# FofanovLab/mtsv_tools

Measured on AMD Instinct MI355X. Metric: reads/sec (whole node), 150bp reads vs MG-index, higher is better.
Workload: dtype u32/i16

## Files before the change

mtsv_tools_amd/csrc/batch.hip:

```cpp
#include <atomic>
#include <chrono>
#include <cmath>
#include <condition_variable>
#include <exception>
#include <mutex>
#include <thread>
#include <cstdio>
#include <cstdlib>
#include <cstring>
#include <stdexcept>
#include <vector>

#include "../../include/mtsv_amd.h"
#include "batch.hpp"
#include "kernels.hpp"

namespace mtsv {

namespace {
template <class F>
void parallel_ranges(uint64_t n, F f) {
    static const int max_nt = [] {
        const char* e = getenv("MTSV_COPY_THREADS");
        return e ? std::max(1, std::min(16, atoi(e))) : 4;
// ... 102 lines not shown
    dev_alloc(&d_out_off, ns + 1, &bytes);
    dev_alloc(&d_tile_sums, (uint64_t)scan_tiles((uint32_t)ns) + 1, &bytes);
    dev_alloc(&d_counters, kCounters, &bytes);
    alloc_hit_workspace();
    dev_alloc(&d_hits, hits_cap, &bytes);
    HIP_CHECK(hipHostMalloc((void**)&h_counters, kCounters * sizeof(uint64_t), hipHostMallocMapped));
    if (const char* e = getenv("MTSV_SW")) sw_pairs = strcmp(e, "packed") != 0;
    if (const char* e = getenv("MTSV_SW_DIAG")) sw_diag = atoi(e) != 0;
    if (const char* e = getenv("MTSV_SW_PREPASS")) sw_prepass = atoi(e) != 0;
    if (const char* e = getenv("MTSV_SW_TOP")) sw_top = atoi(e) != 0;
    if (const char* e = getenv("MTSV_SW_BOUND")) sw_bound = atoi(e) != 0;
    if (const char* e = getenv("MTSV_SW_FUSED")) sw_fused = atoi(e) != 0;
    verify_mode = g_default_verify_mode;
    if (const char* e = getenv("MTSV_VERIFY")) verify_mode = !strcmp(e, "edit_first") ? 1 : 0;
    for (auto& e : ev) HIP_CHECK(hipEventCreate(&e));
    for (int k = 1; k < n_lanes; k++) {
        extra.emplace_back(new Batch(ix, di, ws_reads, 0, hit_cap_user, this));
        bytes += extra.back()->bytes;
    }
}

Batch::~Batch() {
    extra.clear();
    (void)hipSetDevice(di->device);
    (void)hipStreamSynchronize(stream);
    for (void* p : {(void*)d_bases, (void*)d_read_off, (void*)d_seed_lo, (void*)d_seed_cnt, (void*)d_seed_pre, (void*)d_strand_hits,
                    (void*)d_strand_nseeds, (void*)d_strand_off, (void*)d_strand_ncand, (void*)d_worklist,
                    (void*)d_strand_nout, (void*)d_out_off, (void*)d_tile_sums, (void*)d_counters, (void*)d_hit_row,
                    (void*)d_hit_ref, (void*)d_hit_q, (void*)d_hit_key, (void*)d_cand_tmp, (void*)d_cand, (void*)d_out,
                    (void*)d_hits, (void*)d_cand_next, (void*)d_cand_status, (void*)d_heavy_list})
        (void)hipFree(p);
    (void)hipFree(d_codes);
    (void)hipFree(d_strip);
    if (h_hits_stage) pinned_hits_release(h_hits_stage);
    if (copy_stream2) (void)hipStreamDestroy(copy_stream2);
    if (copy_stream) {
        (void)hipStreamSynchronize(copy_stream);
        (void)hipStreamDestroy(copy_stream);
    }
    for (auto& ar : arena) {
        (void)hipFree(ar.d_bases);
        (void)hipFree(ar.d_packed);
        (void)hipFree(ar.d_off);
    }
    if (h_off_all) (void)hipHostFree(h_off_all);
    for (auto& hs : h_stage)
        if (hs) (void)hipHostFree(hs);
    for (auto& e : chunk_ev) (void)hipEventDestroy(e);
    (void)hipHostFree(h_counters);
    for (auto& e : ev) (void)hipEventDestroy(e);
    (void)hipStreamDestroy(stream);
}

void Batch::alloc_hit_workspace() {
    dev_alloc(&d_hit_row, hit_cap, &bytes);
    dev_alloc(&d_hit_ref, hit_cap, &bytes);
    dev_alloc(&d_hit_q, hit_cap, &bytes);
    dev_alloc(&d_hit_key, hit_cap, &bytes);
    dev_alloc(&d_cand_tmp, 2 * hit_cap, &bytes);
    dev_alloc(&d_cand, hit_cap, &bytes);
    dev_alloc(&d_out, hit_cap, &bytes);
    dev_alloc(&d_cand_next, hit_cap, &bytes);
    dev_alloc(&d_cand_status, hit_cap, &bytes);
    dev_alloc(&d_worklist, hit_cap, &bytes);
}

// ... 219 lines not shown
    while (r0 < n_slice) {
        uint32_t nr = (uint32_t)std::min<uint64_t>(pass_reads, n_slice - r0);
        uint32_t pass_max_len = slice_max_len;
        bool tiled = false;
        if (mixed) {
            auto len_of = [&](uint64_t i) { return h_off[i + 1] - h_off[i]; };
            tiled = len_of(r0) > kMaxRegisterReadLen;
            uint32_t cnt = 0, ml = 0;
            while (cnt < nr && (len_of(r0 + cnt) > kMaxRegisterReadLen) == tiled) {
                const uint32_t ml2 = std::max(ml, len_of(r0 + cnt));
                if (tiled && cnt && 2ull * (cnt + 1) * (ml2 >= K ? (ml2 - K) / G + 1 : 0) > kLongPassSlots) break;
                ml = ml2;
                cnt++;
            }
            nr = cnt;
            pass_max_len = ml;
        }
        const uint32_t max_ns = pass_max_len >= K ? (pass_max_len - K) / G + 1 : 0;
        const uint32_t nstr = nr * 2;
        const uint64_t slots = (uint64_t)nstr * max_ns;
        if (slots > seed_cap) {
            (void)hipFree(d_seed_lo);
            (void)hipFree(d_seed_cnt);
            (void)hipFree(d_seed_pre);
            d_seed_lo = d_seed_cnt = d_seed_pre = nullptr;
            const uint64_t want = tiled ? slots : std::max<uint64_t>(slots, 2 * ws_reads * (uint64_t)max_ns);
            uint64_t dummy = 0;
            if (getenv("MTSV_TRACE")) fprintf(stderr, "[workspace] seed slot arrays grow %llu -> %llu entries\n", (unsigned long long)seed_cap, (unsigned long long)want);
            dev_alloc(&d_seed_lo, want, &dummy);
            dev_alloc(&d_seed_cnt, want, &dummy);
            dev_alloc(&d_seed_pre, want, &dummy);
            seed_cap = want;
        }
        HIP_CHECK(hipEventRecord(ev[0], stream));
        const uint32_t listed_cap = (uint32_t)std::min<uint64_t>(slots, std::max<uint64_t>(4096, (uint64_t)((double)slots * listed_share)));
        launch_search(stream, v, sb, so, (uint32_t)r0, nr, max_ns, K, G, d_seed_lo, d_seed_cnt, d_seed_pre, (uint32_t*)(d_counters + 22), listed_cap);
        HIP_CHECK(hipEventRecord(ev[1], stream));
        if (max_ns)
            launch_thin(stream, sb, so, (uint32_t)r0, nr, p.edit_rate, p.min_seed, max_ns, K, G, p.max_hits, p.tune_max_hits, d_seed_cnt,
                        d_seed_pre, d_strand_hits, d_strand_nseeds);
        else {
            HIP_CHECK(hipMemsetAsync(d_strand_hits, 0, (uint64_t)nstr * 4, stream));
            HIP_CHECK(hipMemsetAsync(d_strand_nseeds, 0, (uint64_t)nstr * 4, stream));
        }
        launch_scan(stream, d_strand_hits, nstr, d_tile_sums, d_counters + 0, d_strand_off);
        launch_publish(stream, d_counters, h_counters, 1);
        launch_publish(stream, d_counters + 22, h_counters + 22, 1);
        HIP_CHECK(hipEventRecord(ev[2], stream));
        HIP_CHECK(hipStreamSynchronize(stream));
        {
            const uint64_t n_listed = h_counters[22] & 0xffffffffull;
            const double share = slots ? (double)n_listed / (double)slots : 0.0;
            if (n_listed > listed_cap) {
                listed_share = std::min(1.0, share * 1.25 + 0.01);
                if (getenv("MTSV_TRACE")) fprintf(stderr, "[lane] %llu listed seed slots, grid for %u: pass again\n", (unsigned long long)n_listed, listed_cap);
                continue;
            }
            listed_share = std::min(1.0, std::max(0.02, share * 1.5 + 0.005));
        }
        const uint64_t total_hits = h_counters[0];
        if (total_hits > hit_cap) {
            if (nr > 1) {
                pass_reads = std::max<uint64_t>(1, nr / 2);
                continue;
            }
            if (total_hits > 0xfffffff0ull)
                throw std::runtime_error("device: one read has " + std::to_string(total_hits) + " seed hits, more than 2^32");
            grow_hit_workspace(total_hits);
        }
        stats.n_passes++;
        stats.n_seed_slots += slots;
        stats.n_seed_hits += total_hits;
        launch_expand(stream, v, nstr, max_ns, G, d_seed_lo, d_seed_cnt, d_seed_pre, d_strand_off, d_hit_row, d_hit_ref,
                      d_hit_q);
        HIP_CHECK(hipEventRecord(ev[3], stream));
        if (!v.sa_full)
            launch_locate(stream, v, (uint32_t)total_hits, d_strand_off + nstr, d_hit_row, d_hit_ref,
                          (unsigned long long*)(d_counters + 2));
        HIP_CHECK(hipEventRecord(ev[4], stream));
        HIP_CHECK(hipMemsetAsync(d_counters + 1, 0, 8, stream));
        HIP_CHECK(hipMemsetAsync(d_counters + 7, 0, 8, stream));
        HIP_CHECK(hipMemsetAsync(d_counters + 15, 0, 8, stream));
        launch_coalesce(stream, v, so, (uint32_t)r0, nstr, p.max_candidates, d_strand_off,
                        d_strand_nseeds, d_hit_ref, d_hit_q, d_hit_key, d_cand_tmp, d_cand, d_cand_next,
                        d_cand_status, d_strand_ncand, d_worklist, d_heavy_list, d_counters);
        HIP_CHECK(hipEventRecord(ev[5], stream));
        {
            EvalArgs a;
            a.bases = sb;
            a.read_off = so;
            a.r0 = (uint32_t)r0;
            a.edit_rate = p.edit_rate;
            a.max_candidates = p.max_candidates;
            a.strand_off = d_strand_off;
            a.cand = d_cand;
            a.cand_next = d_cand_next;
            a.cand_status = d_cand_status;
            a.out = d_out;
            a.n_verified = (unsigned long long*)(d_counters + 4);
            a.window_bytes = (unsigned long long*)(d_counters + 5);
            a.sw_columns = (unsigned long long*)(d_counters + 14);
            a.worklist = d_worklist;
            a.wl_count = (const uint32_t*)(d_counters + 1);
            a.wl_cursor = (uint32_t*)(d_counters + 7);
            stats.n_rounds = 1;
            if (tiled) {
                HIP_CHECK(hipMemsetAsync(d_counters + 13, 0, sizeof(uint64_t), stream));
                launch_max_window(stream, nstr, d_strand_off, d_strand_ncand, d_cand, (unsigned long long*)(d_counters + 13));
                launch_publish(stream, d_counters + 13, h_counters + 13, 1);
                HIP_CHECK(hipStreamSynchronize(stream));
                const uint32_t strip_len = (uint32_t)std::max<uint64_t>(h_counters[13], 1);
                const uint64_t need = (uint64_t)tiled_groups(total_hits, strip_len) * strip_len;
                if (need > strip_cap) {
                    (void)hipFree(d_strip);
                    d_strip = nullptr;
                    uint64_t dummy = 0;
                    dev_alloc(&d_strip, need, &dummy);
                    strip_cap = need;
                }
                a.strip = d_strip;
                a.strip_len = strip_len;
                launch_evaluate_tiled(stream, v, a, total_hits);
            } else if (verify_mode == 1 && pass_max_len <= 253) {
                launch_edit_myers(stream, v, a, total_hits, pass_max_len);
            } else if (sw_pairs && pass_max_len <= 253 && hit_cap < 0x80000000ull) {
                const bool fused = sw_bound && sw_fused;
                uint32_t* pass_list = (uint32_t*)d_hit_key;
                uint32_t* sweep_list = (uint32_t*)d_hit_key + hit_cap;
                uint32_t* next_lists[2] = {(uint32_t*)d_cand_tmp, (uint32_t*)d_cand_tmp + hit_cap};
                const uint32_t* wl = d_worklist;
// ... 711 lines not shown
```

mtsv_tools_amd/csrc/batch.hpp:

```cpp
#pragma once
#include <memory>
#include <mutex>
#include <vector>

#include "../../include/mtsv_amd.h"
#include "host_pack.hpp"
#include "dev_index.hpp"
#include "kernels.hpp"

namespace mtsv {

struct Batch {
    mtsv_index* ix;
    DeviceIndex* di;
    hipStream_t stream = nullptr, copy_stream2 = nullptr;
    mtsv_hit* h_hits_stage = nullptr;
    uint64_t h_hits_cap = 0, staged_hits = 0, last_total_hits = 0;
    bool staged_valid = false;
    struct Arena {
        uint8_t* d_bases = nullptr;
        uint8_t* d_packed = nullptr;
        uint32_t* d_off = nullptr;
        uint64_t cap_bases = 0, cap_reads = 0;
    };
// ... 8 lines not shown
    std::vector<hipEvent_t> chunk_ev;
    std::mutex* commit_mu = nullptr;
    uint64_t max_reads, max_bases, hit_cap, hits_cap = 0;
    uint64_t bytes = 0;
    Batch* parent = nullptr;
    std::vector<std::unique_ptr<Batch>> extra;
    int n_lanes = 1;
    uint64_t ws_reads = 0;
    struct Segment {
        Batch* lane;
        uint64_t offset, count;
    };
    std::vector<Segment> segments;
    uint64_t total_hits = 0;
    double run_t0 = 0;
    uint64_t lanes_used = 1;

    uint8_t* d_codes = nullptr;
    uint8_t* d_bases = nullptr;
    uint32_t* d_read_off = nullptr;
    uint32_t *d_seed_lo = nullptr, *d_seed_cnt = nullptr, *d_seed_pre = nullptr;
    uint64_t seed_cap = 0;
    uint32_t *d_strand_hits = nullptr, *d_strand_nseeds = nullptr, *d_strand_off = nullptr, *d_strand_ncand = nullptr,
             *d_worklist = nullptr, *d_strand_nout = nullptr, *d_out_off = nullptr;
    uint64_t* d_tile_sums = nullptr;
    uint64_t* d_counters = nullptr;
    uint32_t *d_hit_row = nullptr, *d_hit_ref = nullptr, *d_hit_q = nullptr;
    uint64_t *d_hit_key = nullptr, *d_cand_tmp = nullptr;
    uint4 *d_cand = nullptr, *d_out = nullptr;
    uint32_t *d_cand_next = nullptr, *d_cand_status = nullptr, *d_heavy_list = nullptr;
    DevHit* d_hits = nullptr;
    uint2* d_strip = nullptr;
    uint64_t strip_cap = 0;
    uint64_t* h_counters = nullptr;
    hipEvent_t ev[15];
    float sw_ms_acc = 0, sweep_ms_acc = 0, diag_ms_acc = 0, bound_ms_acc = 0, edit_ms_acc = 0;
    uint64_t sw_passed_acc = 0;

    std::vector<uint32_t> h_read_off;
    uint32_t max_len = 0;
    static constexpr int kCounters = 24;
    double listed_share = 0.125;
    bool sw_diag = true;
    bool sw_top = true;
    bool sw_bound = true;
    bool sw_fused = true;
    bool sw_prepass = true;
    bool sw_pairs = true;
    int verify_mode = 0;
    uint64_t n_reads = 0;
    uint64_t n_hits_total = 0;
    mtsv_batch_stats stats{};
    float stage_acc[MTSV_N_STAGES] = {0};

    Batch(mtsv_index* ix, DeviceIndex* di, uint64_t max_reads, uint64_t max_bases, uint64_t hit_cap, Batch* parent = nullptr, int lanes = 0);
    ~Batch();
    Batch(const Batch&) = delete;
    Batch& operator=(const Batch&) = delete;

    void upload(const uint8_t* bases, const uint64_t* read_off, uint64_t n);
    void run(const mtsv_params& p);
    void run_host(const uint8_t* bases, const uint64_t* read_off, uint64_t n, const mtsv_params& p, uint64_t read_base = 0);
    struct HostPart {
        const uint8_t* bases;
        const uint64_t* read_off;
        uint64_t n;
// ... 40 lines not shown
```

mtsv_tools_amd/csrc/k_seed.hip:

```cpp
#include "kernels_common.hpp"

namespace mtsv {

namespace {

__device__ inline uint32_t fast_code(uint32_t ch);
__global__ __launch_bounds__(256) void k_normalise(const uint8_t* src, uint8_t* dst, uint64_t lo, uint64_t hi) {
    const uint64_t i = (lo & ~15ull) + ((uint64_t)blockIdx.x * blockDim.x + threadIdx.x) * 16;
    if (i >= hi) return;
    if (i < lo || i + 16 > hi) {
        const uint64_t a = i < lo ? lo : i, b = i + 16 > hi ? hi : i + 16;
        for (uint64_t q = a; q < b; q++) dst[q] = (uint8_t)fast_code(src[q]);
        return;
    }
    uint4 v = *reinterpret_cast<const uint4*>(src + i);
    uint32_t w[4] = {v.x, v.y, v.z, v.w};
#pragma unroll
    for (int k = 0; k < 4; k++) {
        uint32_t o = 0;
#pragma unroll
        for (int q = 0; q < 4; q++) o |= fast_code((w[k] >> (8 * q)) & 0xffu) << (8 * q);
        w[k] = o;
    }
    *reinterpret_cast<uint4*>(dst + i) = make_uint4(w[0], w[1], w[2], w[3]);
// ... 329 lines not shown
        }
    }
    __syncthreads();
    uint32_t at = 0;
    if (lane == 0 && n_slow) at = atomicAdd(&tail_n, n_slow);
    at = __builtin_amdgcn_readfirstlane(at);
    if (lane < n_slow) tail_q[at + lane] = slow_q[lane];
    __syncthreads();
    const uint32_t nt = tail_n;
    if (nt) {
        __shared__ uint32_t tail_base;
        if (threadIdx.x == 0) tail_base = atomicAdd(slow_count, nt);
        __syncthreads();
        if (threadIdx.x < nt) slow_list[tail_base + threadIdx.x] = tail_q[threadIdx.x];
    }
}

__global__ __launch_bounds__(256) void k_search_listed(DevIndexView ix, const uint8_t* __restrict__ bases,
                                                       const uint32_t* __restrict__ read_off, uint32_t r0, uint32_t max_ns, uint32_t K,
                                                       uint32_t G, const uint32_t* __restrict__ slow_list,
                                                       const uint32_t* __restrict__ slow_count, uint32_t* __restrict__ seed_lo,
                                                       uint32_t* __restrict__ seed_cnt) {
    const uint32_t i = blockIdx.x * blockDim.x + threadIdx.x;
    if (i >= *slow_count) return;
    search_slot(ix, bases, read_off, r0, max_ns, K, G, slow_list[i], seed_lo, seed_cnt);
}


__global__ __launch_bounds__(256) void k_thin(const uint8_t* __restrict__ bases, const uint32_t* __restrict__ read_off,
                                              uint32_t r0, uint32_t n_reads, double edit_rate, double min_seed,
                                              uint32_t max_ns, uint32_t K, uint32_t G, uint64_t max_hits,
                                              uint64_t tune_max_hits, uint32_t* __restrict__ seed_cnt,
                                              uint32_t* __restrict__ seed_pre, uint32_t* __restrict__ strand_hits,
                                              uint32_t* __restrict__ strand_nseeds) {
    uint32_t rs = blockIdx.x * blockDim.x + threadIdx.x;
    if (rs >= n_reads * 2) return;
    uint32_t r = r0 + (rs >> 1);
    const uint32_t b0 = read_off[r];
    uint32_t L = read_off[r + 1] - b0;
    uint32_t ns = n_seeds_of(L, K, G);
    uint64_t next_offset = 0, seed_interval = G;
    uint32_t total = 0, nseeds = 0;
    uint32_t* cnt = seed_cnt + (uint64_t)rs * max_ns;
    uint32_t* pre = seed_pre + (uint64_t)rs * max_ns;
    for (uint32_t j = 0; j < ns; j++) {
        uint64_t offset = (uint64_t)j * G;
        const uint32_t raw = cnt[j];
        const uint32_t c = raw == kSeedAtPos ? 1u : raw;
        if (offset < next_offset) {
            if (c) cnt[j] = 0;
            continue;
        }
        if (c == 0) continue;
        if ((uint64_t)c > max_hits) {
            cnt[j] = 0;
            continue;
        }
        if ((uint64_t)c > tune_max_hits) {
            seed_interval *= 2;
            next_offset = offset + seed_interval;
        }
        pre[j] = total;
        total += c;
        nseeds++;
    }
    {
        const bool need = total != 0;
        const int other_need = __shfl_xor((int)need, 1);
        const bool pair_need = need || other_need != 0;
        const uint32_t ED = (uint32_t)ceil((double)L * edit_rate);
        bool hopeless = 2ull * ED > (uint64_t)L;
        uint32_t nn = 0;
        if (pair_need && !hopeless) {
            const uint4* b128 = reinterpret_cast<const uint4*>(bases);
            const uint32_t q0 = b0 >> 4, q1 = (b0 + L + 15) >> 4;
            auto masked = [&](uint32_t qi) {
                const uint4 v = b128[qi];
                const uint32_t w[4] = {v.x, v.y, v.z, v.w};
                uint32_t cnt = 0;
#pragma unroll
                for (int k = 0; k < 4; k++) {
                    const uint32_t byte0 = qi * 16 + 4 * k;
                    uint32_t m = (w[k] >> 2) & 0x01010101u;
                    const int lo = (int)b0 - (int)byte0, hi = (int)(b0 + L) - (int)byte0;
                    if (lo > 0) m = lo >= 4 ? 0u : (m & (0xffffffffu << (8 * lo)));
                    if (hi < 4) m = hi <= 0 ? 0u : (m & ((1u << (8 * hi)) - 1u));
                    cnt += __popc(m);
                }
                return cnt;
            };
            const uint32_t half = rs & 1, ng = q1 - q0;
            if (ng >= 1 && half == 0) nn += masked(q0);
            if (ng >= 2 && half == ((ng - 1) & 1)) nn += masked(q1 - 1);
            for (uint32_t g = half ? 1 : 2; g + 1 < ng; g += 2) {
                const uint4 v = b128[q0 + g];
                nn += __popc((v.x >> 2) & 0x01010101u) + __popc((v.y >> 2) & 0x01010101u) + __popc((v.z >> 2) & 0x01010101u) +
                      __popc((v.w >> 2) & 0x01010101u);
            }
        }
        nn += (uint32_t)__shfl_xor((int)nn, 1);
        hopeless = hopeless || nn > ED;
        const double ms = floor((double)nseeds * min_seed);
        const uint32_t min_seeds = ms < 1.0 ? 1u : (ms > 65535.0 ? 65535u : (uint32_t)ms);
        nseeds = min_seeds | (ED << 16) | ((need && hopeless) ? kHopeless : 0u);
    }
    strand_hits[rs] = total;
    strand_nseeds[rs] = nseeds;
}

constexpr int kScanThreads = 256;
constexpr int kScanItems = 8;
constexpr int kScanTile = kScanThreads * kScanItems;

__device__ inline uint32_t wave_incl_scan(uint32_t v) {
    for (int d = 1; d < kWave; d <<= 1) {
        uint32_t o = __shfl_up(v, d);
        if ((int)lane_id() >= d) v += o;
    }
    return v;
}

__global__ __launch_bounds__(kScanThreads) void k_scan_tile_sums(const uint32_t* __restrict__ in, uint32_t n,
                                                                 uint64_t* __restrict__ tile_sums) {
    __shared__ uint32_t ws[kScanThreads / kWave];
    uint32_t base = blockIdx.x * kScanTile + threadIdx.x * kScanItems;
    uint32_t s = 0;
    for (int i = 0; i < kScanItems; i++)
        if (base + i < n) s += in[base + i];
    for (int d = 32; d > 0; d >>= 1) s += __shfl_down(s, d);
    if (lane_id() == 0) ws[threadIdx.x / kWave] = s;
// ... 186 lines not shown
    (void)hipMemsetAsync(slow_count, 0, sizeof(uint32_t), s);
    uint64_t total = (uint64_t)n_reads * 2 * max_ns;
    if (!total) return;
    const bool fast = ix.kmer_tab && total < 0xffffffffull && K >= 16 && K <= 24 && ix.kmer_k >= 12 && ix.kmer_k <= 17 &&
                      K >= ix.kmer_k && K - std::min<uint32_t>(ix.kmer_k, 16) <= 8 && !getenv("MTSV_SEARCH_GENERIC");
    if (!fast) {
        hipLaunchKernelGGL(k_search, dim3(cdiv(total, 256)), dim3(256), 0, s, ix, bases, read_off, r0, n_reads, max_ns, K, G,
                           seed_lo, seed_cnt);
        return;
    }
    const dim3 grid(std::min<uint32_t>(cdiv(total, 256), 256 * 16));
#define FAST_CASE(KKV)                                                                                                  \
    if (K - KKV > 2)                                                                                                    \
        hipLaunchKernelGGL((k_search_fast<KKV, true>), grid, dim3(256), 0, s, ix, bases, read_off, r0, (uint32_t)total, max_ns, K, G, \
                           seed_lo, seed_cnt, slow_list, slow_count);                                                   \
    else                                                                                                                \
        hipLaunchKernelGGL((k_search_fast<KKV, false>), grid, dim3(256), 0, s, ix, bases, read_off, r0, (uint32_t)total, max_ns, K, G, \
                           seed_lo, seed_cnt, slow_list, slow_count)
    switch (ix.kmer_k) {
    case 12: FAST_CASE(12); break;
    case 13: FAST_CASE(13); break;
    case 14: FAST_CASE(14); break;
    case 15: FAST_CASE(15); break;
    case 17: FAST_CASE(17); break;
    default: FAST_CASE(16); break;
    }
#undef FAST_CASE
    hipLaunchKernelGGL(k_search_listed, dim3(cdiv(std::max<uint32_t>(listed_cap, 1), 256)), dim3(256), 0, s, ix, bases, read_off, r0, max_ns, K, G,
                       slow_list, slow_count, seed_lo, seed_cnt);
}

void launch_thin(hipStream_t s, const uint8_t* bases, const uint32_t* read_off, uint32_t r0, uint32_t n_reads, double edit_rate,
                 double min_seed, uint32_t max_ns, uint32_t K, uint32_t G, uint64_t max_hits, uint64_t tune, uint32_t* seed_cnt, uint32_t* seed_pre,
                 uint32_t* strand_hits, uint32_t* strand_nseeds) {
    hipLaunchKernelGGL(k_thin, dim3(cdiv((uint64_t)n_reads * 2, 256)), dim3(256), 0, s, bases, read_off, r0, n_reads, edit_rate,
                       min_seed, max_ns, K, G, max_hits, tune, seed_cnt, seed_pre, strand_hits, strand_nseeds);
}

void launch_scan(hipStream_t s, const uint32_t* in, uint32_t n, uint64_t* tile_sums, uint64_t* total, uint32_t* out) {
    uint32_t tiles = cdiv(n ? n : 1, kScanTile);
    hipLaunchKernelGGL(k_scan_tile_sums, dim3(tiles), dim3(kScanThreads), 0, s, in, n, tile_sums);
    hipLaunchKernelGGL(k_scan_sums, dim3(1), dim3(1024), 0, s, tile_sums, tiles, total);
    hipLaunchKernelGGL(k_scan_apply, dim3(tiles), dim3(kScanThreads), 0, s, in, n, tile_sums, total, out);
}
uint32_t scan_tiles(uint32_t n) { return cdiv(n ? n : 1, kScanTile); }

void launch_expand(hipStream_t s, const DevIndexView& ix, uint32_t n_strands, uint32_t max_ns, uint32_t G,
                   const uint32_t* seed_lo, const uint32_t* seed_cnt, const uint32_t* seed_pre, const uint32_t* strand_off,
                   uint32_t* hit_row, uint32_t* hit_ref, uint32_t* hit_q) {
    uint64_t n_slots = (uint64_t)n_strands * max_ns;
    if (!n_slots) return;
    hipLaunchKernelGGL(k_expand, dim3(cdiv(n_slots, 256)), dim3(256), 0, s, ix, n_slots, max_ns, G, seed_lo, seed_cnt, seed_pre,
                       strand_off, hit_row, hit_ref, hit_q);
}

void launch_locate(hipStream_t s, const DevIndexView& ix, uint32_t total_hits_host, const uint32_t* total_hits_dev,
                   const uint32_t* hit_row, uint32_t* hit_ref, unsigned long long* lf_steps) {
    if (!total_hits_host) return;
    uint32_t chunks = cdiv(total_hits_host, kLocateChunk);
    uint32_t blocks = std::min<uint32_t>(cdiv(chunks, 4), 256 * 8);
    hipLaunchKernelGGL(k_locate, dim3(blocks), dim3(256), 0, s, ix, total_hits_dev, hit_row, hit_ref, lf_steps);
}

}
```

mtsv_tools_amd/csrc/k_verify.hip:

```cpp
#include "kernels_common.hpp"

namespace mtsv {

namespace {

typedef short pk16 __attribute__((ext_vector_type(2)));

__device__ inline pk16 pk(int lo, int hi) {
    pk16 r;
    r.x = (short)lo;
    r.y = (short)hi;
    return r;
}
__device__ inline pk16 pk_max(pk16 a, pk16 b) { return __builtin_elementwise_max(a, b); }
__device__ inline int pk_bits(pk16 a) { return __builtin_bit_cast(int, a); }
__device__ inline pk16 pk_from_bits(int u) { return __builtin_bit_cast(pk16, u); }

constexpr uint32_t kGroup = 16;
constexpr uint32_t kRing = 1024;

__device__ inline int row_shr1(int v) { return __builtin_amdgcn_update_dpp(0, v, 0x111, 0xf, 0xf, true); }

__device__ inline uint32_t group_ballot(bool p, uint32_t group) { return (uint32_t)(__ballot(p) >> (group * kGroup)) & 0xffffu; }

// ... 1077 lines not shown
    if (!strand) {
        r = load16(ix.text, ix.n, start + j0);
    } else if (end >= j0 + 16) {
        const uint4 v = load16(ix.text, ix.n, end - j0 - 16);
        r.x = __builtin_amdgcn_perm(0, v.w, 0x00010203u);
        r.y = __builtin_amdgcn_perm(0, v.z, 0x00010203u);
        r.z = __builtin_amdgcn_perm(0, v.y, 0x00010203u);
        r.w = __builtin_amdgcn_perm(0, v.x, 0x00010203u);
    } else {
        uint32_t w[4] = {0, 0, 0, 0};
        for (uint32_t i = 0; i < 16; i++) {
            const uint32_t code = end >= j0 + 1 + i ? ix.text[end - j0 - 1 - i] : 7u;
            w[i >> 2] |= code << (8 * (i & 3));
        }
        r = make_uint4(w[0], w[1], w[2], w[3]);
    }
    r.x = sw_matches ? clamp_codes_sw(r.x) : clamp_codes4(r.x);
    r.y = sw_matches ? clamp_codes_sw(r.y) : clamp_codes4(r.y);
    r.z = sw_matches ? clamp_codes_sw(r.z) : clamp_codes4(r.z);
    r.w = sw_matches ? clamp_codes_sw(r.w) : clamp_codes4(r.w);
    return r;
}

enum : int { MY_CHAIN = 0, MY_LIST = 1, MY_BOUND = 2, MY_FUSED = 3 };
template <int W, int MODE>
__global__ __launch_bounds__(256) void k_edit_myers(DevIndexView ix, EvalArgs a) {
    constexpr bool FUSED = MODE == MY_FUSED, LIST = MODE == MY_LIST || FUSED, BOUND = MODE == MY_BOUND;
    constexpr int NROW = (BOUND || LIST) ? 6 : 5;
    __shared__ uint32_t eq_tab[NROW][W][256];
    const uint32_t tid = threadIdx.x;
    const uint32_t n_work = *a.wl_count;
    const uint32_t maxc = a.maxc;
    const uint32_t lane = lane_id();
    const uint32_t* bases32 = reinterpret_cast<const uint32_t*>(a.bases);
    uint32_t verified = 0, wbytes = 0;
    uint32_t cols = 0, refuted = 0;
    uint32_t bnext = 0, bend = 0;
    bool active = false, exhausted = false;
    bool counted = false;
    uint32_t g = 0, o = 0, L = 0, ED = 0, strand = 0;
    bool thr_wrapped = false, hopeless = false;
    uint32_t pv0[W];
    uint32_t ph = 0, extra_passed = 0;
    bool read_n = false;
    for (;;) {
        unsigned long long need = __ballot(!active);
        if (need) {
            if (bnext == bend && !exhausted) {
                const uint32_t n_waves = gridDim.x * (256 / kWave);
                const uint32_t claim = min(256u, max(64u, (n_work / n_waves + 63u) & ~63u));
                uint32_t base = 0;
                if (lane == 0) base = atomicAdd(a.wl_cursor, claim);
                base = __builtin_amdgcn_readfirstlane(base);
                bnext = min(base, n_work);
                bend = min(base + claim, n_work);
                exhausted = bnext == bend;
            }
            const uint32_t take = bnext + __popcll(need & ((1ull << lane) - 1));
            if (!active && take < bend) {
                g = a.worklist[FUSED && a.wl_reverse ? n_work - 1 - take : take];
                if (BOUND) {
                    counted = (g & kSweepFlag) != 0;
                    g &= ~kSweepFlag;
                }
                const uint32_t rs = a.cand[g].w;
                const uint32_t r_ = a.r0 + (rs >> 1);
                strand = rs & 1;
                o = a.strand_off[rs];
                const uint32_t b0 = a.read_off[r_];
                L = a.read_off[r_ + 1] - b0;
                ED = (uint32_t)ceil((double)L * a.edit_rate);
                thr_wrapped = 2ull * ED > (uint64_t)L;
                const int pad = 32 * W - (int)L;
                uint32_t matchable = 0;
#pragma unroll
                for (int k = 0; k < W; k++) {
                    const int q0 = 32 * k - pad;
                    uint32_t mA = 0, mC = 0, mG = 0, mT = 0, wild = 0;
                    if (q0 + 31 >= 0) {
                        const long long byte0 = (long long)b0 + q0;
                        const uint32_t sh = (uint32_t)(byte0 & 3), dsel = (uint32_t)(byte0 >> 2) & 3u;
                        const long long q16 = byte0 >> 4;
                        const uint4* bases128 = reinterpret_cast<const uint4*>(bases32);
                        const uint4 zero4 = make_uint4(0, 0, 0, 0);
                        const uint4 l0 = q16 >= 0 ? bases128[q16] : zero4, l1 = q16 + 1 >= 0 ? bases128[q16 + 1] : zero4,
                                    l2 = q16 + 2 >= 0 ? bases128[q16 + 2] : zero4;
                        const uint32_t dd[12] = {l0.x, l0.y, l0.z, l0.w, l1.x, l1.y, l1.z, l1.w, l2.x, l2.y, l2.z, l2.w};
                        uint32_t d[9];
#pragma unroll
                        for (int j = 0; j < 9; j++) d[j] = dsel == 0 ? dd[j] : dsel == 1 ? dd[j + 1] : dsel == 2 ? dd[j + 2] : dd[j + 3];
#pragma unroll
                        for (int j = 0; j < 8; j++) {
                            const uint32_t four = __builtin_amdgcn_alignbyte(d[j + 1], d[j], sh);
#pragma unroll
                            for (int q = 0; q < 4; q++) {
                                const int bit_i = 4 * j + q;
                                const uint32_t code = (four >> (8 * q)) & 0xffu;
                                const uint32_t bit = 1u << bit_i;
                                const bool real = q0 + bit_i >= 0;
                                mA |= (real && code == 0) ? bit : 0u;
                                mC |= (real && code == 1) ? bit : 0u;
                                mG |= (real && code == 2) ? bit : 0u;
                                mT |= (real && code == 3) ? bit : 0u;
                                wild |= real ? 0u : bit;
                            }
                        }
                    } else {
                        wild = 0xffffffffu;
                    }
                    matchable += __popc(mA | mC | mG | mT);
                    eq_tab[0][k][tid] = (strand ? mT : mA) | wild;
                    eq_tab[1][k][tid] = (strand ? mG : mC) | wild;
                    eq_tab[2][k][tid] = (strand ? mC : mG) | wild;
                    eq_tab[3][k][tid] = (strand ? mA : mT) | wild;
                    eq_tab[4][k][tid] = wild;
                    if (NROW == 6) eq_tab[5][k][tid] = ~(mA | mC | mG | mT);
                    pv0[k] = ~wild;
                }
                hopeless = thr_wrapped || (!BOUND && L - matchable > ED);
                read_n = L != matchable;
                ph = FUSED ? 1 : 0;
                active = true;
            }
            bnext = min(bnext + (uint32_t)__popcll(need), bend);
        }
        if (!__any(active)) {
            if (exhausted) break;
            continue;
        }
        uint32_t verdict = 0, vg = 0;
        if ((FUSED ? thr_wrapped : !LIST && hopeless) && active) {
            const uint4 c = a.cand[g];
            if (!BOUND || !counted) {
                verified++;
                wbytes += c.y - c.x;
            }
            counted = false;
            a.cand_status[g] = 1;
            const uint32_t nxt = a.cand_next[g];
            if (nxt == 0xffffffffu || nxt >= maxc) active = false;
            else g = o + nxt;
        } else if (active) {
            const uint4 c = a.cand[g];
            uint32_t Pv[W], Mv[W];
#pragma unroll
            for (int k = 0; k < W; k++) {
                Pv[k] = pv0[k];
                Mv[k] = 0;
            }
            const uint32_t Wn = c.y - c.x;
            int score = (int)L, best = (int)L;
            const bool swm = BOUND || (LIST && ph == 1);
            uint4 nxt4 = Wn ? fetch_cols(ix, c.x, c.y, strand, 0, swm) : make_uint4(0, 0, 0, 0);
// ... 269 lines not shown
        else SW_TOP(8);
#undef SW_TOP
        return;
    }
#define SW_CASE(RR)                                                                                                      \
    do {                                                                                                                 \
        const uint32_t grid = std::max<uint32_t>(1, std::min<uint32_t>(cdiv(max_items, 32), 256 * ((RR) > 10 ? 3 : kSwOcc))); \
        a.claim_shift = 0;                                                                                               \
        while ((1ull << a.claim_shift) < (uint64_t)grid * 16 * 2) a.claim_shift++;                                       \
        if (diag) hipLaunchKernelGGL((k_sw_pairs<RR, true>), dim3(grid), dim3(256), 0, s, ix, a);                        \
        else hipLaunchKernelGGL((k_sw_pairs<RR, false>), dim3(grid), dim3(256), 0, s, ix, a);                            \
    } while (0)
    if (max_len <= 64) SW_CASE(4);
    else if (max_len <= 96) SW_CASE(6);
    else if (max_len <= 128) SW_CASE(8);
    else if (max_len <= 160) SW_CASE(10);
    else if (max_len <= 208) SW_CASE(13);
    else SW_CASE(16);
#undef SW_CASE
}

void launch_sw_diag(hipStream_t s, const DevIndexView& ix, const EvalArgs& a, uint64_t max_items, uint32_t max_len,
                    uint32_t* sweep_list, uint32_t sweep_slot) {
    const uint32_t grid = std::max<uint32_t>(16, std::min<uint32_t>(cdiv(max_items, 16 * 32), 256 * 6));
    if (max_len <= 128) hipLaunchKernelGGL(k_sw_diag<2>, dim3(grid), dim3(256), 0, s, ix, a, sweep_list, sweep_slot);
    else if (max_len <= 192) hipLaunchKernelGGL(k_sw_diag<3>, dim3(grid), dim3(256), 0, s, ix, a, sweep_list, sweep_slot);
    else hipLaunchKernelGGL(k_sw_diag<4>, dim3(grid), dim3(256), 0, s, ix, a, sweep_list, sweep_slot);
}

void launch_edit_myers(hipStream_t s, const DevIndexView& ix, const EvalArgs& a_, uint64_t max_items, uint32_t max_len,
                       int mode) {
    EvalArgs a = a_;
    a.maxc = rank_bound(a.max_candidates);
    uint32_t blocks = std::max<uint32_t>(16, std::min<uint32_t>(cdiv(max_items, 4096), 256 * 5));
    uint32_t W = (max_len + 31) / 32;
#define MYERS_CASE(WW)                                                                                   \
    do {                                                                                                 \
        if (mode == MY_LIST) hipLaunchKernelGGL((k_edit_myers<WW, MY_LIST>), dim3(blocks), dim3(256), 0, s, ix, a);        \
        else if (mode == MY_FUSED) hipLaunchKernelGGL((k_edit_myers<WW, MY_FUSED>), dim3(blocks), dim3(256), 0, s, ix, a); \
        else if (mode == MY_BOUND) hipLaunchKernelGGL((k_edit_myers<WW, MY_BOUND>), dim3(blocks), dim3(256), 0, s, ix, a); \
        else hipLaunchKernelGGL((k_edit_myers<WW, MY_CHAIN>), dim3(blocks), dim3(256), 0, s, ix, a);                      \
    } while (0)
    if (W <= 2) MYERS_CASE(2);
    else if (W <= 3) MYERS_CASE(3);
    else if (W <= 4) MYERS_CASE(4);
    else if (W <= 5) MYERS_CASE(5);
    else if (W <= 6) MYERS_CASE(6);
    else if (W <= 7) MYERS_CASE(7);
    else MYERS_CASE(8);
#undef MYERS_CASE
}

void launch_resolve(hipStream_t s, uint32_t n_strands, int64_t max_candidates, int64_t max_assignments,
                    const uint32_t* strand_off, const uint32_t* strand_ncand, const uint32_t* cand_status, uint4* out,
                    uint32_t* strand_nout) {
    hipLaunchKernelGGL(k_resolve, dim3(cdiv(n_strands, 256)), dim3(256), 0, s, n_strands, max_candidates, max_assignments,
                       strand_off, strand_ncand, cand_status, out, strand_nout);
}

void launch_gather(hipStream_t s, uint32_t n_strands, uint64_t r0, const uint32_t* strand_off, const uint32_t* strand_nout,
                   const uint32_t* out_off, const uint4* out, DevHit* hits, uint64_t hits_base) {
    hipLaunchKernelGGL(k_gather, dim3(cdiv(n_strands, 256)), dim3(256), 0, s, n_strands, r0, strand_off, strand_nout,
                       out_off, out, hits, hits_base);
}

}
```

mtsv_tools_amd/csrc/kernels.hpp:

```cpp
#pragma once
#include <algorithm>

#include "dev_layout.hpp"

namespace mtsv {

struct DevHit {
    uint64_t read;
    uint32_t tax_id;
    uint32_t gi;
    uint32_t edit;
    uint8_t strand;
    uint8_t pad[3];
    uint64_t offset;
};
static_assert(sizeof(DevHit) == 32, "DevHit must match mtsv_hit");

constexpr uint32_t kCtrVerified = 4, kCtrWindowBytes = 5, kCtrSwCursor = 8, kCtrPassCount = 9, kCtrSwCellPairs = 14;

struct EvalArgs {
    const uint8_t* bases;
    const uint32_t* read_off;
    uint32_t r0;
    double edit_rate;
    int64_t max_candidates;
    const uint32_t* strand_off;
    const uint4* cand;
    const uint32_t* cand_next;
    uint32_t* cand_status;
    const uint32_t* worklist;
    const uint32_t* wl_count;
    uint32_t* wl_cursor;
    uint32_t wl_reverse = 0;
    uint64_t* counters = nullptr;
    uint32_t wl_count_slot = 0;
    uint4* out;
    unsigned long long* n_verified;
    unsigned long long* window_bytes;
    unsigned long long* sw_columns = nullptr;
    uint32_t* pass_list = nullptr;
    uint32_t* pass_count = nullptr;
    uint32_t* next_list = nullptr;
    uint32_t* next_count = nullptr;
    unsigned long long* myers_ctr = nullptr;
    uint32_t* und_list = nullptr;
    uint32_t und_slot = 0;
    uint2* strip = nullptr;
    uint32_t strip_len = 0;
    uint32_t maxc = 0xffffffffu;
    uint32_t claim_shift = 0;
};

constexpr uint32_t kMaxRegisterReadLen = 256;
constexpr uint32_t kMaxReadLen = 32767;

void launch_publish(hipStream_t s, const uint64_t* src, uint64_t* dst_host, uint32_t n);
void launch_normalise(hipStream_t s, const uint8_t* src, uint8_t* dst, uint64_t begin, uint64_t end);
void launch_unpack(hipStream_t s, const uint8_t* packed, uint8_t* dst, uint64_t lo, uint64_t hi);
void launch_search(hipStream_t s, const DevIndexView& ix, const uint8_t* bases, const uint32_t* read_off, uint32_t r0,
                   uint32_t n_reads, uint32_t max_ns, uint32_t K, uint32_t G, uint32_t* seed_lo, uint32_t* seed_cnt,
                   uint32_t* slow_list, uint32_t* slow_count, uint32_t listed_cap);
void launch_thin(hipStream_t s, const uint8_t* bases, const uint32_t* read_off, uint32_t r0, uint32_t n_reads, double edit_rate,
                 double min_seed, uint32_t max_ns, uint32_t K, uint32_t G, uint64_t max_hits, uint64_t tune, uint32_t* seed_cnt, uint32_t* seed_pre,
                 uint32_t* strand_hits, uint32_t* strand_nseeds);
void launch_scan(hipStream_t s, const uint32_t* in, uint32_t n, uint64_t* tile_sums, uint64_t* total, uint32_t* out);
uint32_t scan_tiles(uint32_t n);
void launch_expand(hipStream_t s, const DevIndexView& ix, uint32_t n_strands, uint32_t max_ns, uint32_t G,
                   const uint32_t* seed_lo, const uint32_t* seed_cnt, const uint32_t* seed_pre, const uint32_t* strand_off,
                   uint32_t* hit_row, uint32_t* hit_ref, uint32_t* hit_q);
void launch_locate(hipStream_t s, const DevIndexView& ix, uint32_t total_hits_host, const uint32_t* total_hits_dev,
                   const uint32_t* hit_row, uint32_t* hit_ref, unsigned long long* lf_steps);
void launch_coalesce(hipStream_t s, const DevIndexView& ix, const uint32_t* read_off, uint32_t r0, uint32_t n_strands,
                     int64_t max_candidates, const uint32_t* strand_off,
                     const uint32_t* strand_nseeds, const uint32_t* hit_ref, const uint32_t* hit_q, uint64_t* hit_key,
                     uint64_t* cand_tmp, uint4* cand, uint32_t* cand_next, uint32_t* cand_status,
                     uint32_t* strand_ncand, uint32_t* worklist, uint32_t* heavy_list, uint64_t* counters);
void launch_evaluate(hipStream_t s, const DevIndexView& ix, const EvalArgs& a, uint64_t max_items, uint32_t max_len);
void launch_evaluate_tiled(hipStream_t s, const DevIndexView& ix, const EvalArgs& a, uint64_t max_items);
uint32_t tiled_groups(uint64_t max_items, uint32_t strip_len);
void launch_max_window(hipStream_t s, uint32_t n_strands, const uint32_t* strand_off, const uint32_t* strand_ncand,
                       const uint4* cand, unsigned long long* out);
void launch_edit_myers(hipStream_t s, const DevIndexView& ix, const EvalArgs& a, uint64_t max_items, uint32_t max_len,
                       int mode = 0);
void launch_sw_pairs(hipStream_t s, const DevIndexView& ix, const EvalArgs& a, uint64_t max_items, uint32_t max_len,
                     bool diag = true, bool top = false, bool sparse = false);
void launch_sw_diag(hipStream_t s, const DevIndexView& ix, const EvalArgs& a, uint64_t max_items, uint32_t max_len,
                    uint32_t* sweep_list, uint32_t sweep_slot);
void launch_resolve(hipStream_t s, uint32_t n_strands, int64_t max_candidates, int64_t max_assignments,
                    const uint32_t* strand_off, const uint32_t* strand_ncand, const uint32_t* cand_status, uint4* out,
                    uint32_t* strand_nout);
void launch_gather(hipStream_t s, uint32_t n_strands, uint64_t r0, const uint32_t* strand_off, const uint32_t* strand_nout,
                   const uint32_t* out_off, const uint4* out, DevHit* hits, uint64_t hits_base);

}
```

Measured before the change: 382.8 million.

## Precompute per-read bit-plane images in thin kernel for Myers verification

The thin kernel now packs each read into three 32-bit bit-planes (two code bits plus an N-plane), using DPP lane exchange between strand-pair lanes, and writes them to a new per-read device buffer. The Myers edit kernel then builds its Peq masks from these planes with funnel shifts instead of reloading and byte-decoding the read bases for every candidate. The N-count used for the hopeless check moves from a popcount over read bytes to the N-plane, and hopeless reads are no longer skipped in the thin pass. This adds a plane buffer, extra global writes in the thin kernel, and a hard dependency on the planes being present whenever the Myers path runs.

```diff
diff --git a/mtsv_tools_amd/csrc/batch.hip b/mtsv_tools_amd/csrc/batch.hip
--- a/mtsv_tools_amd/csrc/batch.hip
+++ b/mtsv_tools_amd/csrc/batch.hip
@@ -158,6 +158,7 @@
         (void)hipFree(p);
     (void)hipFree(d_codes);
     (void)hipFree(d_strip);
+    (void)hipFree(d_planes);
     if (h_hits_stage) pinned_hits_release(h_hits_stage);
     if (copy_stream2) (void)hipStreamDestroy(copy_stream2);
     if (copy_stream) {
@@ -443,13 +444,23 @@
             dev_alloc(&d_seed_pre, want, &dummy);
             seed_cap = want;
         }
+        const bool myers_pass = !tiled && pass_max_len <= 253 && (verify_mode == 1 || (sw_pairs && hit_cap < 0x80000000ull));
+        const uint32_t plane_words = myers_pass ? myers_words(pass_max_len) : 0;
+        if ((uint64_t)nr * 3 * plane_words > plane_cap) {
+            (void)hipFree(d_planes);
+            d_planes = nullptr;
+            const uint64_t want = std::max<uint64_t>(nr, ws_reads) * 3 * plane_words;
+            uint64_t dummy = 0;
+            dev_alloc(&d_planes, want, &dummy);
+            plane_cap = want;
+        }
         HIP_CHECK(hipEventRecord(ev[0], stream));
         const uint32_t listed_cap = (uint32_t)std::min<uint64_t>(slots, std::max<uint64_t>(4096, (uint64_t)((double)slots * listed_share)));
         launch_search(stream, v, sb, so, (uint32_t)r0, nr, max_ns, K, G, d_seed_lo, d_seed_cnt, d_seed_pre, (uint32_t*)(d_counters + 22), listed_cap);
         HIP_CHECK(hipEventRecord(ev[1], stream));
         if (max_ns)
             launch_thin(stream, sb, so, (uint32_t)r0, nr, p.edit_rate, p.min_seed, max_ns, K, G, p.max_hits, p.tune_max_hits, d_seed_cnt,
-                        d_seed_pre, d_strand_hits, d_strand_nseeds);
+                        d_seed_pre, d_strand_hits, d_strand_nseeds, myers_pass ? d_planes : nullptr, plane_words);
         else {
             HIP_CHECK(hipMemsetAsync(d_strand_hits, 0, (uint64_t)nstr * 4, stream));
             HIP_CHECK(hipMemsetAsync(d_strand_nseeds, 0, (uint64_t)nstr * 4, stream));
@@ -507,6 +518,8 @@
             a.cand = d_cand;
             a.cand_next = d_cand_next;
             a.cand_status = d_cand_status;
+            a.planes = myers_pass ? d_planes : nullptr;
+            a.plane_words = plane_words;
             a.out = d_out;
             a.n_verified = (unsigned long long*)(d_counters + 4);
             a.window_bytes = (unsigned long long*)(d_counters + 5);
diff --git a/mtsv_tools_amd/csrc/batch.hpp b/mtsv_tools_amd/csrc/batch.hpp
--- a/mtsv_tools_amd/csrc/batch.hpp
+++ b/mtsv_tools_amd/csrc/batch.hpp
@@ -64,6 +64,8 @@
     DevHit* d_hits = nullptr;
     uint2* d_strip = nullptr;
     uint64_t strip_cap = 0;
+    uint32_t* d_planes = nullptr;
+    uint64_t plane_cap = 0;
     uint64_t* h_counters = nullptr;
     hipEvent_t ev[15];
     float sw_ms_acc = 0, sweep_ms_acc = 0, diag_ms_acc = 0, bound_ms_acc = 0, edit_ms_acc = 0;
diff --git a/mtsv_tools_amd/csrc/k_seed.hip b/mtsv_tools_amd/csrc/k_seed.hip
--- a/mtsv_tools_amd/csrc/k_seed.hip
+++ b/mtsv_tools_amd/csrc/k_seed.hip
@@ -385,7 +385,8 @@
                                               uint32_t max_ns, uint32_t K, uint32_t G, uint64_t max_hits,
                                               uint64_t tune_max_hits, uint32_t* __restrict__ seed_cnt,
                                               uint32_t* __restrict__ seed_pre, uint32_t* __restrict__ strand_hits,
-                                              uint32_t* __restrict__ strand_nseeds) {
+                                              uint32_t* __restrict__ strand_nseeds, uint32_t* __restrict__ planes,
+                                              uint32_t plane_words) {
     uint32_t rs = blockIdx.x * blockDim.x + threadIdx.x;
     if (rs >= n_reads * 2) return;
     uint32_t r = r0 + (rs >> 1);
@@ -424,31 +425,60 @@
         const uint32_t ED = (uint32_t)ceil((double)L * edit_rate);
         bool hopeless = 2ull * ED > (uint64_t)L;
         uint32_t nn = 0;
-        if (pair_need && !hopeless) {
+        if (pair_need) {
             const uint4* b128 = reinterpret_cast<const uint4*>(bases);
             const uint32_t q0 = b0 >> 4, q1 = (b0 + L + 15) >> 4;
-            auto masked = [&](uint32_t qi) {
-                const uint4 v = b128[qi];
-                const uint32_t w[4] = {v.x, v.y, v.z, v.w};
-                uint32_t cnt = 0;
-#pragma unroll
-                for (int k = 0; k < 4; k++) {
-                    const uint32_t byte0 = qi * 16 + 4 * k;
-                    uint32_t m = (w[k] >> 2) & 0x01010101u;
-                    const int lo = (int)b0 - (int)byte0, hi = (int)(b0 + L) - (int)byte0;
-                    if (lo > 0) m = lo >= 4 ? 0u : (m & (0xffffffffu << (8 * lo)));
-                    if (hi < 4) m = hi <= 0 ? 0u : (m & ((1u << (8 * hi)) - 1u));
-                    cnt += __popc(m);
-                }
-                return cnt;
-            };
-            const uint32_t half = rs & 1, ng = q1 - q0;
-            if (ng >= 1 && half == 0) nn += masked(q0);
-            if (ng >= 2 && half == ((ng - 1) & 1)) nn += masked(q1 - 1);
-            for (uint32_t g = half ? 1 : 2; g + 1 < ng; g += 2) {
-                const uint4 v = b128[q0 + g];
-                nn += __popc((v.x >> 2) & 0x01010101u) + __popc((v.y >> 2) & 0x01010101u) + __popc((v.z >> 2) & 0x01010101u) +
-                      __popc((v.w >> 2) & 0x01010101u);
+            const uint32_t half = rs & 1, sh = b0 & 15u, nw = (L + 31) >> 5;
+            uint32_t* img = planes ? planes + ((uint64_t)(rs >> 1) * plane_words) * 3 : nullptr;
+            uint32_t a0 = 0, a1 = 0, an = 0;
+            constexpr uint32_t kAhead = 3;
+            for (uint32_t i0 = 0; i0 <= nw; i0 += kAhead) {
+              uint4 vb[kAhead];
+#pragma unroll
+              for (uint32_t u = 0; u < kAhead; u++) {
+                  const uint32_t q = q0 + 2 * (i0 + u) + half;
+                  vb[u] = make_uint4(0, 0, 0, 0);
+                  if (i0 + u <= nw && q < q1) vb[u] = b128[q];
+              }
+#pragma unroll
+              for (uint32_t u = 0; u < kAhead; u++) {
+                const uint32_t i = i0 + u;
+                if (i > nw) break;
+                const uint4 v = vb[u];
+                uint32_t h01 = 0, hn = 0;
+                {
+                    const uint32_t c0 = (v.x & 0x07070707u) | ((v.y & 0x07070707u) << 4);
+                    const uint32_t c1 = (v.z & 0x07070707u) | ((v.w & 0x07070707u) << 4);
+                    auto gather = [](uint32_t y) {
+                        y &= 0x11111111u;
+                        y |= y >> 7;
+                        y |= y >> 14;
+                        return y & 0xffu;
+                    };
+                    h01 = gather(c0) | (gather(c1) << 8) | (gather(c0 >> 1) << 16) | (gather(c1 >> 1) << 24);
+                    hn = gather(c0 >> 2) | (gather(c1 >> 2) << 8);
+                }
+                const uint32_t o01 = (uint32_t)__builtin_amdgcn_update_dpp(0, (int)h01, 0xB1, 0xf, 0xf, false);
+                const uint32_t on = (uint32_t)__builtin_amdgcn_update_dpp(0, (int)hn, 0xB1, 0xf, 0xf, false);
+                const uint32_t lo01 = half ? o01 : h01, hi01 = half ? h01 : o01;
+                const uint32_t c0 = (lo01 & 0xffffu) | (hi01 << 16), c1 = (lo01 >> 16) | (hi01 & 0xffff0000u);
+                const uint32_t cn = half ? (on | (hn << 16)) : (hn | (on << 16));
+                if (i && ((i - 1) & 1) == half) {
+                    const uint32_t w = i - 1, left = L - 32 * w;
+                    const uint32_t m = left >= 32 ? 0xffffffffu : (1u << left) - 1u;
+                    const uint32_t w0 = __builtin_amdgcn_alignbit(c0, a0, sh) & m, w1 = __builtin_amdgcn_alignbit(c1, a1, sh) & m,
+                                   wn = __builtin_amdgcn_alignbit(cn, an, sh) & m;
+                    nn += __popc(wn);
+                    if (img) {
+                        img[3 * w] = w0;
+                        img[3 * w + 1] = w1;
+                        img[3 * w + 2] = wn;
+                    }
+                }
+                a0 = c0;
+                a1 = c1;
+                an = cn;
+              }
             }
         }
         nn += (uint32_t)__shfl_xor((int)nn, 1);
@@ -701,9 +731,9 @@
 
 void launch_thin(hipStream_t s, const uint8_t* bases, const uint32_t* read_off, uint32_t r0, uint32_t n_reads, double edit_rate,
                  double min_seed, uint32_t max_ns, uint32_t K, uint32_t G, uint64_t max_hits, uint64_t tune, uint32_t* seed_cnt, uint32_t* seed_pre,
-                 uint32_t* strand_hits, uint32_t* strand_nseeds) {
+                 uint32_t* strand_hits, uint32_t* strand_nseeds, uint32_t* planes, uint32_t plane_words) {
     hipLaunchKernelGGL(k_thin, dim3(cdiv((uint64_t)n_reads * 2, 256)), dim3(256), 0, s, bases, read_off, r0, n_reads, edit_rate,
-                       min_seed, max_ns, K, G, max_hits, tune, seed_cnt, seed_pre, strand_hits, strand_nseeds);
+                       min_seed, max_ns, K, G, max_hits, tune, seed_cnt, seed_pre, strand_hits, strand_nseeds, planes, plane_words);
 }
 
 void launch_scan(hipStream_t s, const uint32_t* in, uint32_t n, uint64_t* tile_sums, uint64_t* total, uint32_t* out) {
diff --git a/mtsv_tools_amd/csrc/k_verify.hip b/mtsv_tools_amd/csrc/k_verify.hip
--- a/mtsv_tools_amd/csrc/k_verify.hip
+++ b/mtsv_tools_amd/csrc/k_verify.hip
@@ -1133,7 +1133,6 @@
     const uint32_t n_work = *a.wl_count;
     const uint32_t maxc = a.maxc;
     const uint32_t lane = lane_id();
-    const uint32_t* bases32 = reinterpret_cast<const uint32_t*>(a.bases);
     uint32_t verified = 0, wbytes = 0;
     uint32_t cols = 0, refuted = 0;
     uint32_t bnext = 0, bend = 0;
@@ -1173,53 +1172,39 @@
                 ED = (uint32_t)ceil((double)L * a.edit_rate);
                 thr_wrapped = 2ull * ED > (uint64_t)L;
                 const int pad = 32 * W - (int)L;
-                uint32_t matchable = 0;
+                const uint32_t nw = (L + 31) >> 5, pw = (uint32_t)(pad + 31) >> 5, sh = (uint32_t)(-pad) & 31u;
+                const uint32_t* img = a.planes + ((uint64_t)(rs >> 1) * a.plane_words) * 3;
+                uint32_t P0[W + 1], P1[W + 1], PN[W + 1];
+#pragma unroll
+                for (int j = 0; j <= W; j++) {
+                    const uint32_t idx = (uint32_t)j - pw;
+                    P0[j] = P1[j] = PN[j] = 0;
+                    if (idx < nw) {
+                        P0[j] = img[3 * idx];
+                        P1[j] = img[3 * idx + 1];
+                        PN[j] = img[3 * idx + 2];
+                    }
+                }
+                uint32_t read_ns = 0;
 #pragma unroll
                 for (int k = 0; k < W; k++) {
-                    const int q0 = 32 * k - pad;
-                    uint32_t mA = 0, mC = 0, mG = 0, mT = 0, wild = 0;
-                    if (q0 + 31 >= 0) {
-                        const long long byte0 = (long long)b0 + q0;
-                        const uint32_t sh = (uint32_t)(byte0 & 3), dsel = (uint32_t)(byte0 >> 2) & 3u;
-                        const long long q16 = byte0 >> 4;
-                        const uint4* bases128 = reinterpret_cast<const uint4*>(bases32);
-                        const uint4 zero4 = make_uint4(0, 0, 0, 0);
-                        const uint4 l0 = q16 >= 0 ? bases128[q16] : zero4, l1 = q16 + 1 >= 0 ? bases128[q16 + 1] : zero4,
-                                    l2 = q16 + 2 >= 0 ? bases128[q16 + 2] : zero4;
-                        const uint32_t dd[12] = {l0.x, l0.y, l0.z, l0.w, l1.x, l1.y, l1.z, l1.w, l2.x, l2.y, l2.z, l2.w};
-                        uint32_t d[9];
-#pragma unroll
-                        for (int j = 0; j < 9; j++) d[j] = dsel == 0 ? dd[j] : dsel == 1 ? dd[j + 1] : dsel == 2 ? dd[j + 2] : dd[j + 3];
-#pragma unroll
-                        for (int j = 0; j < 8; j++) {
-                            const uint32_t four = __builtin_amdgcn_alignbyte(d[j + 1], d[j], sh);
-#pragma unroll
-                            for (int q = 0; q < 4; q++) {
-                                const int bit_i = 4 * j + q;
-                                const uint32_t code = (four >> (8 * q)) & 0xffu;
-                                const uint32_t bit = 1u << bit_i;
-                                const bool real = q0 + bit_i >= 0;
-                                mA |= (real && code == 0) ? bit : 0u;
-                                mC |= (real && code == 1) ? bit : 0u;
-                                mG |= (real && code == 2) ? bit : 0u;
-                                mT |= (real && code == 3) ? bit : 0u;
-                                wild |= real ? 0u : bit;
-                            }
-                        }
-                    } else {
-                        wild = 0xffffffffu;
-                    }
-                    matchable += __popc(mA | mC | mG | mT);
-                    eq_tab[0][k][tid] = (strand ? mT : mA) | wild;
-                    eq_tab[1][k][tid] = (strand ? mG : mC) | wild;
-                    eq_tab[2][k][tid] = (strand ? mC : mG) | wild;
-                    eq_tab[3][k][tid] = (strand ? mA : mT) | wild;
+                    const uint32_t p0 = __builtin_amdgcn_alignbit(P0[k + 1], P0[k], sh), p1 = __builtin_amdgcn_alignbit(P1[k + 1], P1[k], sh),
+                                   pn = __builtin_amdgcn_alignbit(PN[k + 1], PN[k], sh);
+                    const int below = pad - 32 * k;
+                    const uint32_t wild = below >= 32 ? 0xffffffffu : below <= 0 ? 0u : (1u << below) - 1u;
+                    const uint32_t mA = ~(p0 | p1 | pn), mC = (p0 & ~p1 & ~pn) | wild, mG = (p1 & ~p0 & ~pn) | wild,
+                                   mT = (p0 & p1 & ~pn) | wild;
+                    read_ns += __popc(pn);
+                    eq_tab[0][k][tid] = strand ? mT : mA;
+                    eq_tab[1][k][tid] = strand ? mG : mC;
+                    eq_tab[2][k][tid] = strand ? mC : mG;
+                    eq_tab[3][k][tid] = strand ? mA : mT;
                     eq_tab[4][k][tid] = wild;
-                    if (NROW == 6) eq_tab[5][k][tid] = ~(mA | mC | mG | mT);
+                    if (NROW == 6) eq_tab[5][k][tid] = pn | wild;
                     pv0[k] = ~wild;
                 }
-                hopeless = thr_wrapped || (!BOUND && L - matchable > ED);
-                read_n = L != matchable;
+                hopeless = thr_wrapped || (!BOUND && read_ns > ED);
+                read_n = read_ns != 0;
                 ph = FUSED ? 1 : 0;
                 active = true;
             }
@@ -1555,8 +1540,9 @@
                        int mode) {
     EvalArgs a = a_;
     a.maxc = rank_bound(a.max_candidates);
+    if (!a.planes || a.plane_words != myers_words(max_len)) throw std::runtime_error("internal: k_edit_myers needs the pass's read planes");
     uint32_t blocks = std::max<uint32_t>(16, std::min<uint32_t>(cdiv(max_items, 4096), 256 * 5));
-    uint32_t W = (max_len + 31) / 32;
+    const uint32_t W = myers_words(max_len);
 #define MYERS_CASE(WW)                                                                                   \
     do {                                                                                                 \
         if (mode == MY_LIST) hipLaunchKernelGGL((k_edit_myers<WW, MY_LIST>), dim3(blocks), dim3(256), 0, s, ix, a);        \
@@ -1564,12 +1550,12 @@
         else if (mode == MY_BOUND) hipLaunchKernelGGL((k_edit_myers<WW, MY_BOUND>), dim3(blocks), dim3(256), 0, s, ix, a); \
         else hipLaunchKernelGGL((k_edit_myers<WW, MY_CHAIN>), dim3(blocks), dim3(256), 0, s, ix, a);                      \
     } while (0)
-    if (W <= 2) MYERS_CASE(2);
-    else if (W <= 3) MYERS_CASE(3);
-    else if (W <= 4) MYERS_CASE(4);
-    else if (W <= 5) MYERS_CASE(5);
-    else if (W <= 6) MYERS_CASE(6);
-    else if (W <= 7) MYERS_CASE(7);
+    if (W == 2) MYERS_CASE(2);
+    else if (W == 3) MYERS_CASE(3);
+    else if (W == 4) MYERS_CASE(4);
+    else if (W == 5) MYERS_CASE(5);
+    else if (W == 6) MYERS_CASE(6);
+    else if (W == 7) MYERS_CASE(7);
     else MYERS_CASE(8);
 #undef MYERS_CASE
 }
diff --git a/mtsv_tools_amd/csrc/kernels.hpp b/mtsv_tools_amd/csrc/kernels.hpp
--- a/mtsv_tools_amd/csrc/kernels.hpp
+++ b/mtsv_tools_amd/csrc/kernels.hpp
@@ -47,9 +47,13 @@
     uint32_t und_slot = 0;
     uint2* strip = nullptr;
     uint32_t strip_len = 0;
+    const uint32_t* planes = nullptr;
+    uint32_t plane_words = 0;
     uint32_t maxc = 0xffffffffu;
     uint32_t claim_shift = 0;
 };
+
+inline uint32_t myers_words(uint32_t max_len) { return std::min(std::max((max_len + 31) / 32, 2u), 8u); }
 
 constexpr uint32_t kMaxRegisterReadLen = 256;
 constexpr uint32_t kMaxReadLen = 32767;
@@ -62,7 +66,7 @@
                    uint32_t* slow_list, uint32_t* slow_count, uint32_t listed_cap);
 void launch_thin(hipStream_t s, const uint8_t* bases, const uint32_t* read_off, uint32_t r0, uint32_t n_reads, double edit_rate,
                  double min_seed, uint32_t max_ns, uint32_t K, uint32_t G, uint64_t max_hits, uint64_t tune, uint32_t* seed_cnt, uint32_t* seed_pre,
-                 uint32_t* strand_hits, uint32_t* strand_nseeds);
+                 uint32_t* strand_hits, uint32_t* strand_nseeds, uint32_t* planes, uint32_t plane_words);
 void launch_scan(hipStream_t s, const uint32_t* in, uint32_t n, uint64_t* tile_sums, uint64_t* total, uint32_t* out);
 uint32_t scan_tiles(uint32_t n);
 void launch_expand(hipStream_t s, const DevIndexView& ix, uint32_t n_strands, uint32_t max_ns, uint32_t G,
```

New measurement: 394.6 million, median of 6. 1.03x the previous value.
